# RupertLuo/Valley

Hardware: NVIDIA H100
Metric: generated tokens/s (8-frame video requests: ViT-L/14 encode + pool/project + LLaMA prefill + 256 greedy tokens per sequence) (higher is better)
Workload: dtype bf16

## Files before the change

### include/valley_b200.h

```cpp
#ifndef VALLEY_B200_H_
#define VALLEY_B200_H_

#include <stdint.h>

#ifdef __cplusplus
extern "C" {
#endif

typedef struct vly_ctx vly_ctx;
typedef struct vly_kv vly_kv;

typedef enum {
  VLY_OK = 0,
  VLY_ERR_INVALID = -1,
  VLY_ERR_CUDA = -2,
  VLY_ERR_STATE = -3,
  VLY_ERR_IM_COUNT = -10,
  VLY_ERR_IM_CUT = -11,
  VLY_ERR_INDEX = -12
} vly_status;

typedef enum { VLY_F32 = 0, VLY_BF16 = 1, VLY_F16 = 2 } vly_dtype;

typedef struct {
// ... 103 lines not shown
  float* scores_out;
  float* logits_out;
  int64_t* beam_indices_out;
  int32_t* steps_out;
} vly_beam;

int vly_beam_search(vly_ctx* ctx, vly_kv* kv, const vly_beam* params, const float* first_logits_dev, int prompt_len, int n_steps,
                    int64_t* seq_out_dev, float* scores_out_dev, int* gen_len_out_dev, void* stream);
int vly_kv_beam_reorder(vly_ctx* ctx, vly_kv* kv, const int32_t* parent_rows_dev, int from_pos, void* stream);

int vly_kernel_launch_count(vly_ctx* ctx, int64_t* out);
int vly_held_bytes(int64_t* device_bytes, int64_t* pinned_bytes);
int vly_num_sms(vly_ctx* ctx, int* out);

int vly_kv_debug_counters(vly_kv* kv, long long* host_out, int n);
void vly_set_error_(const char* message);

int vly_test_gemm(vly_ctx* ctx, const void* a_dev, const void* w_dev, int M, int N, int K, int epi, const float* bias_dev,
                  const void* residual_dev, void* out_dev, int block_n, void* stream);
int vly_test_vit_attention(vly_ctx* ctx, const void* qkv_dev, int n_frames, void* out_dev, void* stream);
int vly_test_sample_filter(vly_ctx* ctx, const float* logits_dev, int B, int V, float temperature, int top_k, float top_p,
                           uint8_t* keep_out_dev, void* stream);
int vly_test_stop_strings(vly_ctx* ctx, const vly_sampling* sampling, int V, const int64_t* tokens_dev, int B, int n,
                          uint8_t* out_dev, void* stream);
int vly_test_gemv(vly_ctx* ctx, int mode, const void* w_dev, const void* x_dev, int N, int K, int B, int64_t ldx, float eps,
                  const void* res_dev, void* out_dev, void* kcache_dev, void* vcache_dev, int Smax, int pos, float* logits_dev,
                  int64_t* next_tokens_dev, void* stream);
int vly_test_decode_attention(vly_ctx* ctx, const void* q_dev, const void* kcache_dev, const void* vcache_dev, int B, int nH,
                              int Smax, int len, const uint8_t* key_mask_dev, void* out_dev, void* stream);

// ... 5 lines not shown
```

### valley_b200/_lib.py

```python
from __future__ import annotations

import ctypes as C
import os

_HERE = os.path.dirname(os.path.abspath(__file__))
LIB_PATH = os.environ.get("VLY_LIB_PATH") or os.path.join(_HERE, "lib", "libvalley_b200.so")


class VlyConfig(C.Structure):
    _fields_ = [
        ("hidden_size", C.c_int32), ("num_hidden_layers", C.c_int32), ("num_attention_heads", C.c_int32),
        ("intermediate_size", C.c_int32), ("vocab_size", C.c_int32),
        ("rms_norm_eps", C.c_float), ("rope_theta", C.c_float),
        ("max_position_embeddings", C.c_int32),
        ("vit_hidden", C.c_int32), ("vit_layers", C.c_int32), ("vit_heads", C.c_int32), ("vit_mlp", C.c_int32),
        ("vit_patch", C.c_int32), ("vit_image", C.c_int32),
        ("vit_eps", C.c_float),
        ("mm_vision_select_layer", C.c_int32),
        ("device", C.c_int32),
        ("patch_pooling_method", C.c_int32),
    ]


class VlyTokens(C.Structure):
# ... 78 lines not shown
    "vly_kv_reset": (_i, [_vp, _vp]),
    "vly_kv_set_key_mask": (_i, [_vp, _vp, _i, _vp]),
    "vly_kv_export": (_i, [_vp, _vp, _i, _i, _vp, _vp]),
    "vly_llama_prefill": (_i, [_vp, _vp, _vp, _i, _i, _i, _vp, _vp, _vp]),
    "vly_llama_decode": (_i, [_vp, _vp, _vp, _vp, _vp, _vp]),
    "vly_generate_greedy": (_i, [_vp, _vp, _vp, _i, _vp, _vp]),
    "vly_cross_entropy": (_i, [_vp, _vp, _vp, _i, _i, _i64, _vp, _vp]),
    "vly_sample_logits": (_i, [_vp, _vp, _vp, _p(VlySampling), _vp, _vp]),
    "vly_generate": (_i, [_vp, _vp, _vp, _i, _vp, _p(VlySampling), _vp, _vp]),
    "vly_beam_search": (_i, [_vp, _vp, _p(VlyBeam), _vp, _i, _i, _vp, _vp, _vp, _vp]),
    "vly_kv_beam_reorder": (_i, [_vp, _vp, _vp, _i, _vp]),
    "vly_kernel_launch_count": (_i, [_vp, _p(_i64)]),
    "vly_held_bytes": (_i, [_p(_i64), _p(_i64)]),
    "vly_num_sms": (_i, [_vp, _p(_i)]),
    "vly_kv_debug_counters": (_i, [_vp, _vp, _i]),
    "vly_set_error_": (None, [C.c_char_p]),
    "vly_test_gemm": (_i, [_vp, _vp, _vp, _i, _i, _i, _i, _vp, _vp, _vp, _i, _vp]),
    "vly_test_vit_attention": (_i, [_vp, _vp, _i, _vp, _vp]),
    "vly_test_sample_filter": (_i, [_vp, _vp, _i, _i, C.c_float, _i, C.c_float, _vp, _vp]),
    "vly_test_stop_strings": (_i, [_vp, _p(VlySampling), _i, _vp, _i, _i, _vp, _vp]),
    "vly_test_gemv":(_i, [_vp, _i, _vp, _vp, _i, _i, _i, _i64, C.c_float, _vp, _vp, _vp, _vp, _i, _i, _vp, _vp, _vp]),
    "vly_test_decode_attention": (_i, [_vp, _vp, _vp, _vp, _i, _i, _i, _i, _vp, _vp, _vp]),
}

_lib = None


def load():
    global _lib
    if _lib is not None:
# ... 29 lines not shown
```

### valley_b200/csrc/api.cu

```cuda
#include <cuda_runtime.h>
#include <cuda.h>

#include <algorithm>
#include <atomic>
#include <cmath>
#include <cstdarg>
#include <cstdio>
#include <cstdlib>
#include <cstring>
#include <map>
#include <memory>
#include <mutex>
#include <string>
#include <type_traits>
#include <utility>
#include <vector>

#include "../../include/valley_b200.h"
#include "attention_tc.cuh"
#include "common.cuh"
#include "gemm_tc.cuh"
#include "simt_kernels.cuh"
#include "decode_kernels.cuh"
#include "decode_mega.cuh"
// ... 164 lines not shown
  int* d_step = nullptr;
  Owned<bf16> x, q, attn, hb;
  Owned<float> part_o;
  Owned<float2> part_ml;
  Owned<unsigned int> counters;
  Owned<float> part_val;
  Owned<int> part_idx;
  Owned<float> logits;
  Owned<long long> cur_tokens;
  Owned<long long> gen_tokens;
  int nsplit = 1;
  Owned<PhaseDesc> d_phases;
  StepParams mega = {};
  size_t mega_smem = 0;
  Owned<long long> dbg;
  Owned<SampleState> d_sample;
  bool sample_dirty = false;
  bool filtered = false;
  bool recording = false;
  Owned<uint32_t> key_bits;
  bool masked = false;
  int mask_words() const { return Smax / 32; }
  Owned<BeamState> d_beam;
  Owned<long long> beam_tok;
  Owned<int> beam_bidx;
  Owned<float> beam_div;
  Owned<int> beam_from;
  Owned<uint8_t> stop_buf, stop_stage;
  cudaEvent_t stop_event = nullptr;
  bool stop_ready = false;
// ... 828 lines not shown
  if (!c || !ids || !out || B <= 0 || S <= 0) return fail(VLY_ERR_INVALID, "vly_embed_splice: bad argument");
  if (src_map && (!img_idx || !vis_rows)) return fail(VLY_ERR_INVALID, "vly_embed_splice: src_map given without img_idx / vis_rows");
  std::lock_guard<std::mutex> lk(c->mu);
  if (!c->finalized || !c->has_llm) return fail(VLY_ERR_STATE, "vly_embed_splice: LLM weights not loaded");
  CK(cudaSetDevice(c->cfg.device));
  return launch(c, embed_splice_kernel, {dim3(B * S), dim3(128), 0, (cudaStream_t)stream}, (const long long*)ids, src_map, img_idx, c->embed,
                (const bf16*)vis_rows, rows_per_img, (bf16*)out, nullptr, 0, S, c->cfg.hidden_size, c->cfg.vocab_size);
}

static void mega_smem_layout(const vly_config& g, int bmax, size_t* x_bytes, size_t* misc) {
  const bool tc = bmax > 1;
  const int kmax = g.intermediate_size > g.hidden_size ? g.intermediate_size : g.hidden_size;
  const size_t xs_stride_b = tc ? (size_t)(((kmax * 2 + 127) & ~127) + MegaCfg::PAD_TC) : (size_t)kmax * 2;
  *x_bytes = ((size_t)bmax * xs_stride_b + 127) & ~size_t(127);
  const int nv = (tc ? MegaCfg::ROWS_TC : MegaCfg::ROWS) * bmax;
  *misc = (2 * MegaCfg::MAX_STAGES + 2 * MegaCfg::RED_SLOTS + 2) * 8 + (size_t)MegaCfg::RED_SLOTS * 16 * nv * 4 + (3 + 16) * bmax * 4 + 256;
}
static const size_t kMegaSmem = 226 * 1024;
static const int kMegaDbgCounters = 1024 * 8;

struct DecodeSettings {
  int stage_kb = 0;
  int rows = 0;
  int inflight_kb = 100;
  int stages = 0;
  int inflight = 0;
  int attn_ikeys = 0;
  int l2_hint = 1;
  bool dbg = false;
};
static DecodeSettings read_decode_settings() {
// ... 70 lines not shown
    d.type = PH_ATTN; d.N = 0; d.K = 0; d.W = nullptr; d.x_in = nullptr; d.out = kv->attn; add(d);
    d.type = PH_OPROJ; d.N = H; d.K = H; d.W = w.wo; d.x_in = kv->attn; d.out = kv->x; add(d);
    d.type = PH_GATEUP; d.N = 2 * I; d.K = H; d.W = w.wgu; d.x_in = kv->x; d.out = kv->hb; add(d);
    d.type = PH_DOWN; d.N = H; d.K = I; d.W = w.wdown; d.x_in = kv->hb; d.out = kv->x; add(d);
  }
  {
    PhaseDesc d = {};
    d.type = PH_LOGITS; d.N = V; d.K = H; d.W = c->lm_head; d.x_in = kv->x; d.out = nullptr; add(d);
  }
  stage_bytes = (stage_bytes + 127) & ~127;
  for (PhaseDesc& q : ph) {
    if (q.type == PH_ATTN) continue;
    const int sb = q.rows * (q.kc * 2 + pad);
    q.inflight = (s.inflight_kb * 1024 + sb / 2) / sb;
    if (q.inflight < 2) q.inflight = 2;
  }
  int n_stages = (int)(((long long)kMegaSmem - (long long)x_bytes - (long long)misc) / (long long)stage_bytes);
  if (n_stages > MegaCfg::MAX_STAGES) n_stages = MegaCfg::MAX_STAGES;
  const int cap = s.stages > 0 ? s.stages : 4;
  if (n_stages > cap) n_stages = cap;
  if (n_stages < 2)
    return fail(VLY_ERR_INVALID, "vly_kv_create: activations (B=%d, K=%d) leave no room for the weight ring (%d stages, at least 2 needed)",
                B, std::max(I, H), n_stages);
  if (s.dbg) {
    fprintf(stderr, "[vly] decode ring: B=%d x=%zu B, ring budget %zu B, slot %d B, %d slots fit, %d used;", B, x_bytes, ring_budget,
            stage_bytes, (int)(ring_budget / stage_bytes), n_stages);
    for (int i = 0; i < 5 && i < (int)ph.size(); ++i)
      if (ph[i].type != PH_ATTN) fprintf(stderr, " type%d N=%d K=%d rows=%d kc=%d inflight=%d;", ph[i].type, ph[i].N, ph[i].K, ph[i].rows, ph[i].kc, ph[i].inflight);
    fprintf(stderr, " logits rows=%d kc=%d\n", ph.back().rows, ph.back().kc);
    TRY(kv->dbg.alloc(kMegaDbgCounters * sizeof(long long)));
  }
  TRY(kv->d_phases.alloc(ph.size() * sizeof(PhaseDesc)));
  CK(cudaMemcpy(kv->d_phases, ph.data(), ph.size() * sizeof(PhaseDesc), cudaMemcpyHostToDevice));

  StepParams& p = kv->mega;
  p = {};
  p.phases = kv->d_phases; p.n_phases = (int)ph.size();
  p.B = B; p.H = H; p.nH = nH; p.Smax = kv->Smax; p.V = V;
  p.Kmax = std::max(I, H);
  p.eps = g.rms_norm_eps; p.scale_log2e = 0.08838834764831845f * 1.4426950408889634f;
  p.rope = c->rope; p.seq_len = kv->d_len; p.step = kv->d_step; p.embed = c->embed; p.tokens_in = kv->cur_tokens;
  p.x = kv->x; p.q = kv->q; p.attn = kv->attn;
  p.part_o = kv->part_o; p.part_ml = kv->part_ml; p.attn_counters = kv->counters; p.nsplit = kv->nsplit;
  p.key_bits = kv->key_bits; p.mask_words = kv->mask_words();
  p.logits = kv->logits; p.part_val = kv->part_val; p.part_idx = kv->part_idx;
  p.next_tokens = kv->cur_tokens; p.out_tokens = kv->gen_tokens; p.out_stride = kv->Smax;
  p.sample = kv->d_sample;
  p.grid_counter = kv->counters + (size_t)B * nH + 1;
  p.grid_epoch = p.grid_counter + 1;
  p.n_grid_syncs = p.n_phases + 1;
  p.attn_ikeys = s.attn_ikeys;
  p.n_stages = n_stages;
  p.stage_bytes = stage_bytes;
  p.n_inflight = s.inflight > 0 ? s.inflight : n_stages;
  if (p.n_inflight > n_stages) p.n_inflight = n_stages;
  p.l2_hint = s.l2_hint;
  p.dbg = kv->dbg;
  kv->mega_smem = (size_t)n_stages * stage_bytes + x_bytes + misc;
  return VLY_OK;
}

extern "C" int vly_kv_create(vly_ctx* c, int batch, int max_seq, vly_kv** out) {
  if (!c || !out || batch <= 0 || max_seq <= 0) return fail(VLY_ERR_INVALID, "vly_kv_create: bad argument");
  if (!c->finalized || !c->has_llm) return fail(VLY_ERR_STATE, "vly_kv_create: LLM weights not finalised");
  if (max_seq > c->cfg.max_position_embeddings) return fail(VLY_ERR_INVALID, "vly_kv_create: max_seq %d > max_position_embeddings %d", max_seq, c->cfg.max_position_embeddings);
  CK(cudaSetDevice(c->cfg.device));
  const vly_config& g = c->cfg;
  auto kv = std::make_unique<vly_kv>();
  kv->ctx = c;
  kv->B = batch;
  kv->Smax = (max_seq + 127) / 128 * 128;
  const int H = g.hidden_size, nH = g.num_attention_heads, I = g.intermediate_size, V = g.vocab_size, L = g.num_hidden_layers;
// ... 275 lines not shown
  if (next_tokens_dev) CK(cudaMemcpyAsync(next_tokens_dev, kv->cur_tokens, (size_t)B * 8, cudaMemcpyDeviceToDevice, st));
  kv->host_len = past + S;
  return launch(c, set_int_kernel, {dim3(1), dim3(1), 0, st}, kv->d_len, kv->host_len);
}

extern "C" int vly_kv_debug_counters(vly_kv* kv, long long* host_out, int n) {
  if (!kv || !host_out || n < 0) return fail(VLY_ERR_INVALID, "vly_kv_debug_counters: bad argument");
  if (!kv->dbg)
    return fail(VLY_ERR_STATE, "vly_kv_debug_counters: this cache has no counters (B %d; they need B <= 4 and VLY_MEGA_DBG set when it was created)", kv->B);
  if (n > kMegaDbgCounters) return fail(VLY_ERR_INVALID, "vly_kv_debug_counters: %d values requested, the cache holds %d", n, kMegaDbgCounters);
  CK(cudaSetDevice(kv->ctx->cfg.device));
  CK(cudaMemcpy(host_out, kv->dbg, (size_t)n * sizeof(long long), cudaMemcpyDeviceToHost));
  return VLY_OK;
}

static int launch_decode_mega(vly_ctx* c, vly_kv* kv, bool select, cudaStream_t st) {
  StepParams p = kv->mega;
  p.select = select ? 1 : 0;
  LaunchCfg l = {dim3(c->num_sms), dim3(MegaCfg::THREADS), kv->mega_smem, st};
  l.cooperative = true;
  return with_bmax(kv->B, [&](auto bm) { return launch(c, decode_step_kernel<decltype(bm)::value>, l, p); });
}

static int launch_sample_filter(vly_ctx* c, const float* logits, int B, int V, SampleState* s, const int* seq_len, const int* step,
                                long long* next_tokens, long long* out_tokens, int out_stride, bool filter, bool per_op,
                                uint8_t* keep_out, cudaStream_t st) {
  const size_t smem = filter && (size_t)V * 4 <= (size_t)kFilterStageMaxBytes ? (size_t)V * 4 : 0;
  return launch(c, sample_filter_kernel, {dim3(B), dim3(kFilterThreads), smem, st}, logits, V, s, seq_len, step, next_tokens, out_tokens,
                out_stride, filter ? 1 : 0, per_op ? 1 : 0, keep_out);
}
// ... 515 lines not shown
```

### valley_b200/csrc/decode_mega.cuh

```cuda
#pragma once
#include "common.cuh"
#include "simt_kernels.cuh"
#include "decode_kernels.cuh"
#include "sampling.cuh"

namespace vly {

enum PhaseType : int { PH_QKV = 0, PH_ATTN = 1, PH_OPROJ = 2, PH_GATEUP = 3, PH_DOWN = 4, PH_LOGITS = 5 };

struct PhaseDesc {
  int type, N, K, layer;
  int rows, kc;
  int inflight;
  const __nv_bfloat16* W;
  const __nv_bfloat16* x_in;
  __nv_bfloat16* out;
  __nv_bfloat16* kcache;
  __nv_bfloat16* vcache;
};

struct StepParams {
  const PhaseDesc* phases;
  int n_phases;
  int B, H, nH, Smax, V, Kmax;
  float eps, scale_log2e;
  const float2* rope;
  int* seq_len;
// ... 13 lines not shown
  float* part_val;
  int* part_idx;
  long long* next_tokens;
  long long* out_tokens;
  int out_stride;
  SampleState* sample;
  unsigned int* grid_counter;
  unsigned int* grid_epoch;
  int n_grid_syncs;
  int attn_ikeys;
  int n_stages;
  int stage_bytes;
  int n_inflight;
  int l2_hint;
  long long* dbg;
  int select;
};

struct MegaCfg {
  static constexpr int ROWS = 4;
  static constexpr int ROWS_TC = 8;
  static constexpr int PAD_TC = 64;
  static constexpr int CONSUMERS = 512, THREADS = 576;
  static constexpr int RED_SLOTS = 4;
  static constexpr int MAX_STAGES = 8;
  static constexpr int ATTN_KEYS_MIN = 16;
};

VLY_DEVINL uint4 ldcg_v4(const void* p) {
  uint4 r;
  asm volatile("ld.global.cg.v4.u32 {%0, %1, %2, %3}, [%4];\n" : "=r"(r.x), "=r"(r.y), "=r"(r.z), "=r"(r.w) : "l"(p) : "memory");
  return r;
}
VLY_DEVINL float ldcg_bf16(const __nv_bfloat16* p) {
  unsigned short v;
  asm volatile("ld.global.cg.u16 %0, [%1];\n" : "=h"(v) : "l"(p) : "memory");
  return __uint_as_float((uint32_t)v << 16);
}
VLY_DEVINL void mma_m16n8k16_bf16(float (&d)[4], uint32_t a0, uint32_t a1, uint32_t a2, uint32_t a3, uint32_t b0, uint32_t b1) {
  asm volatile("mma.sync.aligned.m16n8k16.row.col.f32.bf16.bf16.f32 {%0,%1,%2,%3}, {%4,%5,%6,%7}, {%8,%9}, {%0,%1,%2,%3};\n"
               : "+f"(d[0]), "+f"(d[1]), "+f"(d[2]), "+f"(d[3])
               : "r"(a0), "r"(a1), "r"(a2), "r"(a3), "r"(b0), "r"(b1));
}

VLY_DEVINL uint32_t ld_acquire_u32(const unsigned int* p) {
  uint32_t v;
  asm volatile("ld.acquire.gpu.global.u32 %0, [%1];\n" : "=r"(v) : "l"(p) : "memory");
  return v;
}
VLY_DEVINL void fence_proxy_async_global() { asm volatile("fence.proxy.async.global;\n" ::: "memory"); }

VLY_DEVINL void grid_sync_consumers(unsigned int* counter, unsigned int target, int ct) {
  asm volatile("bar.sync 2, 544;" ::: "memory");
  if (ct == 0) {
    asm volatile("red.release.gpu.global.add.u32 [%0], 1;\n" ::"l"(counter) : "memory");
    while ((int)(ld_acquire_u32(counter) - target) < 0) {
    }
  }
  asm volatile("bar.sync 2, 544;" ::: "memory");
}

VLY_DEVINL void mega_attention_phase(const StepParams& p, const PhaseDesc& d, const int cw, const int lane, const int pos) {
  const int len = pos + 1;
  const int n_warps = 16 * (int)gridDim.x;
  int ikeys = p.attn_ikeys;
  if (ikeys == 0) {
    if (p.B * p.nH * ((len + 15) >> 4) <= n_warps) ikeys = 16;
    else
      for (ikeys = 32; ikeys < 256; ikeys += 16)
        if (p.B * p.nH * ((len + ikeys - 1) / ikeys) <= n_warps + n_warps / 20) break;
  }
  const int n_act = (len + ikeys - 1) / ikeys;
  const int items = p.B * p.nH * n_act;
  const int hl = lane & 15, hw = lane >> 4;
// ... 150 lines not shown

VLY_DEVINL void mega_epilogue_prefetch(const StepParams& p, const PhaseDesc& d, const bool ok, const int b, const int n, const int pos,
                                       float& pre0, float& pre1) {
  if (ok) {
    if (d.type == PH_OPROJ || d.type == PH_DOWN) pre0 = ldcg_bf16(d.out + (size_t)b * d.N + n);
    else if (d.type == PH_QKV && n < 2 * p.H) {
      const float2 cs = __ldg(p.rope + (size_t)pos * 64 + ((n & 127) >> 1));
      pre0 = cs.x;
      pre1 = cs.y;
    }
  }
}

template <int BMAX, int NV>
VLY_DEVINL void mega_unit_epilogue(const StepParams& p, const PhaseDesc& d, const int lane, const float t, const bool ok, const int r,
                                   const int b, const int n, const float pre0, const float pre1, const int pos, const float* rstd_s,
                                   float* bestv, int* besti, const bool samp_on, const float samp_it, const uint32_t samp_k0,
                                   const uint32_t samp_k1) {
  constexpr unsigned kMask = (NV == 32) ? 0xffffffffu : ((1u << NV) - 1u);
  if (d.type == PH_OPROJ || d.type == PH_DOWN) {
    if (ok) d.out[(size_t)b * d.N + n] = __float2bfloat16_rn(t + pre0);
  } else if (d.type == PH_LOGITS) {
    const float y = t * rstd_s[b];
    if (ok && p.logits != nullptr) p.logits[(size_t)b * d.N + n] = y;
    float bv = ok ? (samp_on ? sample_score(y, samp_it, samp_k0, samp_k1, n, b, pos) : y) : -INFINITY;
    int bi = n;
#pragma unroll
    for (int o = BMAX; o < NV; o <<= 1) {
      const float ov = __shfl_xor_sync(kMask, bv, o);
      const int oi = __shfl_xor_sync(kMask, bi, o);
      if (ov > bv || (ov == bv && oi < bi)) { bv = ov; bi = oi; }
    }
    if (lane < BMAX && lane < p.B && bv > bestv[lane]) {
      bestv[lane] = bv;
      besti[lane] = bi;
    }
  } else {
    const float mine = t * rstd_s[b];
    const float other = __shfl_xor_sync(kMask, mine, BMAX);
    if ((r & 1) == 0 && ok && n + 1 < d.N) {
      float x0 = mine, x1 = other;
      if (d.type == PH_GATEUP) {
        const float gte = bf16_round(x0), up = bf16_round(x1);
        d.out[(size_t)b * (d.N >> 1) + (n >> 1)] = __float2bfloat16_rn(bf16_round(gte / (1.f + __expf(-gte))) * up);
      } else {
        const int which = n / p.H, nh = n - which * p.H, head = nh >> 7, cidx = nh & 127;
        if (which < 2) {
          const float a = x0 * pre0 - x1 * pre1, c2 = x1 * pre0 + x0 * pre1;
          x0 = a;
          x1 = c2;
        }
        __nv_bfloat16* dst;
        if (which == 0) dst = d.out + (size_t)b * p.H + nh;
// ... 38 lines not shown
  constexpr int ROWS = kTC ? M::ROWS_TC : M::ROWS;
  constexpr int NV = ROWS * BMAX;
  constexpr int PAD = kTC ? M::PAD_TC : 0;
  extern __shared__ uint8_t msm_raw[];
  uint8_t* msm = msm_raw + ((128u - (smem_u32(msm_raw) & 127u)) & 127u);
  uint8_t* ring = msm;
  __nv_bfloat16* xs = reinterpret_cast<__nv_bfloat16*>(ring + (size_t)p.n_stages * p.stage_bytes);
  const int xs_stride = kTC ? (((p.Kmax * 2 + 127) & ~127) + PAD) / 2 : p.Kmax;
  const size_t xs_bytes = ((size_t)BMAX * xs_stride * 2 + 127) & ~size_t(127);
  uint8_t* tail = reinterpret_cast<uint8_t*>(xs) + xs_bytes;
  uint64_t* full_bar = reinterpret_cast<uint64_t*>(tail);
  uint64_t* empty_bar = full_bar + M::MAX_STAGES;
  uint64_t* red_full = empty_bar + M::MAX_STAGES;
  uint64_t* red_empty = red_full + M::RED_SLOTS;
  uint64_t* x_bar = red_empty + M::RED_SLOTS;
  float* red = reinterpret_cast<float*>(x_bar + 2);
  float* rstd_s = red + M::RED_SLOTS * 16 * NV;
  float* bestv = rstd_s + BMAX;
  int* besti = reinterpret_cast<int*>(bestv + BMAX);
  float* wred = reinterpret_cast<float*>(besti + BMAX);

  const int tid = threadIdx.x, warp = tid >> 5, lane = tid & 31;
  if (p.sample->all_done) return;
  if (tid == 0) {
    for (int i = 0; i < p.n_stages; ++i) {
      mbar_init(&full_bar[i], 1);
      mbar_init(&empty_bar[i], 16);
    }
    for (int i = 0; i < M::RED_SLOTS; ++i) {
      mbar_init(&red_full[i], 16);
      mbar_init(&red_empty[i], 1);
    }
    mbar_init(x_bar, 1);
    fence_barrier_init();
  }
  __syncthreads();

  if (warp == 0) {
    if (lane == 0) {
      int st = 0;
      uint32_t ph = 0;
      int wst = 0, issued = 0, confirmed = 0;
      uint32_t wph = 0;
      long long* dbg_p = p.dbg != nullptr ? p.dbg + (size_t)blockIdx.x * 32 : nullptr;
      if (dbg_p != nullptr)
        for (int i = 26; i < 32; ++i) dbg_p[i] = 0;
      const bool hint = p.l2_hint != 0;
      const uint64_t pol_stream = l2_policy_evict_first();
      for (int pi = 0; pi < p.n_phases; ++pi) {
        const PhaseDesc d = p.phases[pi];
        if (d.type == PH_ATTN) continue;
        const int rows_u = d.rows, KCp = d.kc;
        const int row_stride = KCp * 2 + PAD;
        const int n_groups = (d.N + rows_u - 1) / rows_u;
        const int n_slices = (d.K + KCp - 1) / KCp;
        const int infl = min(d.inflight, p.n_inflight);
        long long t_blocked = 0;
        for (int g = blockIdx.x; g < n_groups; g += gridDim.x) {
          const int n0 = g * rows_u;
          const int rows = min(rows_u, d.N - n0);
          for (int s = 0; s < n_slices; ++s) {
            const int kc = min(KCp, d.K - s * KCp);
            const long long t_w = dbg_p != nullptr ? clock64() : 0;
            mbar_wait(&empty_bar[st], ph ^ 1);
            while (issued - confirmed >= infl) {
              mbar_wait(&full_bar[wst], wph);
              if (++wst == p.n_stages) { wst = 0; wph ^= 1; }
              ++confirmed;
            }
            if (dbg_p != nullptr) t_blocked += clock64() - t_w;
            ++issued;
            mbar_expect_tx(&full_bar[st], (uint32_t)rows * kc * 2);
            uint8_t* dst = ring + (size_t)st * p.stage_bytes;
            const __nv_bfloat16* src = d.W + (size_t)n0 * d.K + (size_t)s * KCp;
            if (PAD == 0 && kc == d.K) {
// ... 13 lines not shown
    }
    return;
  }

  const bool is_fin = (warp == 17);
  const int ct = tid - 32;
  const int cw = warp - 1;
  const int pos = *p.seq_len;
  const bool samp_on = p.select && p.sample->enabled != 0;
  const float samp_it = p.sample->inv_temp;
  const uint32_t samp_k0 = p.sample->seed_lo, samp_k1 = p.sample->seed_hi;
  unsigned int sync_no = 0;
  const unsigned int sync_base = *p.grid_epoch * (unsigned int)p.n_grid_syncs * gridDim.x;
  long long t_sync = 0, t_stage = 0, t_loop = 0, t_attn = 0, t0 = clock64();
  long long* dbg_o = (p.dbg != nullptr && ct == 0) ? p.dbg + (size_t)blockIdx.x * 32 : nullptr;
  if (dbg_o != nullptr)
    for (int i = 8; i < 26; ++i) dbg_o[i] = 0;
  {
    if (!is_fin) {
      const int chunks = p.B * (p.H >> 3);
      for (int i = blockIdx.x * M::CONSUMERS + ct; i < chunks; i += gridDim.x * M::CONSUMERS) {
        const int b = i / (p.H >> 3), c = i % (p.H >> 3);
        long long id = p.tokens_in[b];
        id = id < 0 ? 0 : (id >= p.V ? p.V - 1 : id);
        *reinterpret_cast<uint4*>(p.x + (size_t)b * p.H + c * 8) = *reinterpret_cast<const uint4*>(p.embed + (size_t)id * p.H + c * 8);
      }
    } else if (lane < BMAX) {
      bestv[lane] = -INFINITY;
      besti[lane] = 0;
    }
    grid_sync_consumers(p.grid_counter, sync_base + (++sync_no) * gridDim.x, ct);
    t_sync += clock64() - t0;
  }

  int st = 0;
  uint32_t ph = 0, xph = 0;
  unsigned int unit_no = 0;
  for (int pi = 0; pi < p.n_phases; ++pi) {
    const PhaseDesc d = p.phases[pi];
    t0 = clock64();
    if (d.type == PH_ATTN) {
      if (!is_fin) mega_attention_phase(p, d, cw, lane, pos);
      t_attn += clock64() - t0;
      if (dbg_o != nullptr) dbg_o[8 + 3 * PH_ATTN + 1] += clock64() - t0;
    } else {
      const bool norm = (d.type == PH_QKV || d.type == PH_GATEUP || d.type == PH_LOGITS);
      const int rows_u = d.rows, KCp = d.kc;
      const int row_stride = KCp * 2 + PAD;
      if (!is_fin) {
        if (ct == 0) {
          fence_proxy_async_global();
          mbar_expect_tx(x_bar, (uint32_t)p.B * d.K * 2);
          for (int b = 0; b < p.B; ++b) bulk_load_1d(xs + (size_t)b * xs_stride, d.x_in + (size_t)b * d.K, (uint32_t)d.K * 2, x_bar);
        }
        mbar_wait(x_bar, xph);
        if (norm) {
          float sq[BMAX];
#pragma unroll
          for (int b = 0; b < BMAX; ++b) sq[b] = 0.f;
          const int chunks = d.K >> 3;
          for (int c = ct; c < chunks; c += M::CONSUMERS) {
#pragma unroll
            for (int b = 0; b < BMAX; ++b) {
              if (b < p.B) {
                const uint4 w = *reinterpret_cast<const uint4*>(xs + (size_t)b * xs_stride + c * 8);
                const uint32_t ww[4] = {w.x, w.y, w.z, w.w};
#pragma unroll
                for (int i = 0; i < 4; ++i) {
                  const float a = bf16_lo(ww[i]), bb = bf16_hi(ww[i]);
                  sq[b] += a * a + bb * bb;
                }
              }
            }
          }
#pragma unroll
          for (int b = 0; b < BMAX; ++b) {
            const float v = warp_sum(sq[b]);
            if (lane == 0) wred[cw * BMAX + b] = v;
          }
        }
      }
      xph ^= 1;
      if (norm) {
        asm volatile("bar.sync 2, 544;" ::: "memory");
        if (!is_fin && ct < BMAX) {
          float t = 0.f;
          for (int w = 0; w < 16; ++w) t += wred[w * BMAX + ct];
          rstd_s[ct] = rsqrtf(t / d.K + p.eps);
        }
        asm volatile("bar.sync 2, 544;" ::: "memory");
      }
      t_stage += clock64() - t0;
      if (dbg_o != nullptr) dbg_o[8 + 3 * d.type] += clock64() - t0;
      t0 = clock64();
      const int n_groups = (d.N + rows_u - 1) / rows_u;
      const int n_slices = (d.K + KCp - 1) / KCp;
      if (!is_fin) {
        for (int g = blockIdx.x; g < n_groups; g += gridDim.x, ++unit_no) {
          const int n0 = g * rows_u;
          const int rows = min(rows_u, d.N - n0);
          const int slot = unit_no & (M::RED_SLOTS - 1);
          const uint32_t round = (unit_no / M::RED_SLOTS) & 1;
          if constexpr (kTC) {
            const int gq = lane >> 2, tq = lane & 3;
            float dacc[4] = {0.f, 0.f, 0.f, 0.f}, dacc1[4] = {0.f, 0.f, 0.f, 0.f};
            const bool w_ok = gq < rows, x_ok = gq < p.B;
            for (int s = 0; s < n_slices; ++s) {
              const int kc = min(KCp, d.K - s * KCp);
              mbar_wait(&full_bar[st], ph);
              const uint8_t* wrow = ring + (size_t)st * p.stage_bytes + gq * row_stride;
              const __nv_bfloat16* xrow = xs + (size_t)gq * xs_stride + (size_t)s * KCp;
              const int nblk = kc >> 5, bpw = (nblk + 15) >> 4;
              const int kb0 = cw * bpw, kb1 = min(kb0 + bpw, nblk);
#pragma unroll 4
              for (int kb = kb0; kb < kb1; ++kb) {
                const int k = kb << 5;
                uint4 wb = make_uint4(0, 0, 0, 0), xa = make_uint4(0, 0, 0, 0);
                if (w_ok) wb = *reinterpret_cast<const uint4*>(wrow + (k + tq * 8) * 2);
                if (x_ok) xa = *reinterpret_cast<const uint4*>(xrow + k + tq * 8);
                mma_m16n8k16_bf16(dacc, xa.x, 0u, xa.y, 0u, wb.x, wb.y);
                mma_m16n8k16_bf16(dacc1, xa.z, 0u, xa.w, 0u, wb.z, wb.w);
              }
              __syncwarp();
              if (lane == 0) mbar_arrive(&empty_bar[st]);
              if (++st == p.n_stages) { st = 0; ph ^= 1; }
            }
            dacc[0] += dacc1[0];
            dacc[1] += dacc1[1];
            mbar_wait(&red_empty[slot], round ^ 1);
            if (gq < BMAX) {
              float* rp = red + (slot * 16 + cw) * NV;
              rp[(2 * tq) * BMAX + gq] = dacc[0];
              rp[(2 * tq + 1) * BMAX + gq] = dacc[1];
            }
            __syncwarp();
            if (lane == 0) mbar_arrive(&red_full[slot]);
            continue;
          }
          float acc[NV];
#pragma unroll
          for (int i = 0; i < NV; ++i) acc[i] = 0.f;
          for (int s = 0; s < n_slices; ++s) {
            const int kc = min(KCp, d.K - s * KCp);
            mbar_wait(&full_bar[st], ph);
            for (int c8 = ct * 8; c8 < kc; c8 += M::CONSUMERS * 8) {
              const uint8_t* src = ring + (size_t)st * p.stage_bytes + c8 * 2;
              float xf[BMAX][8];
#pragma unroll
              for (int b = 0; b < BMAX; ++b) {
                const uint4 xv = *reinterpret_cast<const uint4*>(xs + (size_t)b * xs_stride + (size_t)s * KCp + c8);
                xf[b][0] = bf16_lo(xv.x); xf[b][1] = bf16_hi(xv.x); xf[b][2] = bf16_lo(xv.y); xf[b][3] = bf16_hi(xv.y);
                xf[b][4] = bf16_lo(xv.z); xf[b][5] = bf16_hi(xv.z); xf[b][6] = bf16_lo(xv.w); xf[b][7] = bf16_hi(xv.w);
              }
#pragma unroll
              for (int r = 0; r < ROWS; ++r) {
                if (r < rows) {
                  const uint4 wv = *reinterpret_cast<const uint4*>(src + r * row_stride);
                  const float wf[8] = {bf16_lo(wv.x), bf16_hi(wv.x), bf16_lo(wv.y), bf16_hi(wv.y),
                                       bf16_lo(wv.z), bf16_hi(wv.z), bf16_lo(wv.w), bf16_hi(wv.w)};
#pragma unroll
                  for (int b = 0; b < BMAX; ++b)
#pragma unroll
                    for (int e = 0; e < 8; ++e) acc[r * BMAX + b] = fmaf(wf[e], xf[b][e], acc[r * BMAX + b]);
                }
              }
            }
            __syncwarp();
            if (lane == 0) mbar_arrive(&empty_bar[st]);
            if (++st == p.n_stages) { st = 0; ph ^= 1; }
          }
          warp_reduce_scatter<NV>(acc, lane);
          mbar_wait(&red_empty[slot], round ^ 1);
          if ((lane & (32 / NV - 1)) == 0) red[(slot * 16 + cw) * NV + lane / (32 / NV)] = acc[0];
          __syncwarp();
          if (lane == 0) mbar_arrive(&red_full[slot]);
        }
      } else {
        for (int g = blockIdx.x; g < n_groups; g += gridDim.x, ++unit_no) {
          const int n0 = g * rows_u;
          const int slot = unit_no & (M::RED_SLOTS - 1);
          const uint32_t round = (unit_no / M::RED_SLOTS) & 1;
          const int r = lane / BMAX, b = lane % BMAX, n = n0 + r;
          const bool ok = lane < NV && r < rows_u && b < p.B && n < d.N;
          float pre0 = 0.f, pre1 = 0.f;
          mega_epilogue_prefetch(p, d, ok, b, n, pos, pre0, pre1);
          mbar_wait(&red_full[slot], round);
          float t = 0.f;
          if (lane < NV) {
#pragma unroll
            for (int w = 0; w < 16; ++w) t += red[(slot * 16 + w) * NV + lane];
          }
          __syncwarp();
          if (lane == 0) mbar_arrive(&red_empty[slot]);
          if (lane < NV)
            mega_unit_epilogue<BMAX, NV>(p, d, lane, t, ok, r, b, n, pre0, pre1, pos, rstd_s, bestv, besti, samp_on, samp_it, samp_k0, samp_k1);
        }
      }
      t_loop += clock64() - t0;
      if (dbg_o != nullptr) dbg_o[8 + 3 * d.type + 1] += clock64() - t0;
    }
    t0 = clock64();
    if (pi == p.n_phases - 1 && is_fin && lane < p.B) {
      p.part_val[(size_t)lane * gridDim.x + blockIdx.x] = bestv[lane];
      p.part_idx[(size_t)lane * gridDim.x + blockIdx.x] = besti[lane];
    }
    grid_sync_consumers(p.grid_counter, sync_base + (++sync_no) * gridDim.x, ct);
    t_sync += clock64() - t0;
    if (dbg_o != nullptr) dbg_o[8 + 3 * d.type + 2] += clock64() - t0;
  }
  if (dbg_o != nullptr) {
    dbg_o[0] = t_sync; dbg_o[1] = t_stage; dbg_o[2] = t_loop; dbg_o[3] = t_attn; dbg_o[4] = 0;
  }

  if (blockIdx.x == 0 && !is_fin) mega_finish_step(p, cw, lane, ct);
}

}
```

Measured before the change: 387.8.

## Overlap activation loads and RMSNorm with GEMV in decode megakernel, balance tail rows

Splits the per-phase activation bulk load into per-K-slice barriers so consumers can start the first unit's GEMV as soon as their slice arrives, instead of waiting for the whole vector. The RMSNorm sum-of-squares moves to after the first unit's reduction and is signalled through a new norm barrier, taking it off the critical path before compute. Row units are reassigned so full rounds use the normal row count and the leftover tail is spread evenly across all SMs, reducing load imbalance in the last round. Also adds globaltimer boundary timestamps for debugging, plus more mbarrier bookkeeping and phase-parity state that has to stay consistent.

```diff
diff --git a/include/valley_b200.h b/include/valley_b200.h
--- a/include/valley_b200.h
+++ b/include/valley_b200.h
@@ -141,6 +141,7 @@
 int vly_num_sms(vly_ctx* ctx, int* out);
 
 int vly_kv_debug_counters(vly_kv* kv, long long* host_out, int n);
+int vly_kv_debug_boundaries(vly_kv* kv, long long* host_out, int n);
 void vly_set_error_(const char* message);
 
 int vly_test_gemm(vly_ctx* ctx, const void* a_dev, const void* w_dev, int M, int N, int K, int epi, const float* bias_dev,
diff --git a/valley_b200/_lib.py b/valley_b200/_lib.py
--- a/valley_b200/_lib.py
+++ b/valley_b200/_lib.py
@@ -116,6 +116,7 @@
     "vly_held_bytes": (_i, [_p(_i64), _p(_i64)]),
     "vly_num_sms": (_i, [_vp, _p(_i)]),
     "vly_kv_debug_counters": (_i, [_vp, _vp, _i]),
+    "vly_kv_debug_boundaries": (_i, [_vp, _vp, _i]),
     "vly_set_error_": (None, [C.c_char_p]),
     "vly_test_gemm": (_i, [_vp, _vp, _vp, _i, _i, _i, _i, _vp, _vp, _vp, _i, _vp]),
     "vly_test_vit_attention": (_i, [_vp, _vp, _i, _vp, _vp]),
diff --git a/valley_b200/csrc/api.cu b/valley_b200/csrc/api.cu
--- a/valley_b200/csrc/api.cu
+++ b/valley_b200/csrc/api.cu
@@ -202,6 +202,8 @@
   StepParams mega = {};
   size_t mega_smem = 0;
   Owned<long long> dbg;
+  Owned<long long> dbg_bnd;
+  size_t dbg_bnd_n = 0;
   Owned<SampleState> d_sample;
   bool sample_dirty = false;
   bool filtered = false;
@@ -1060,7 +1062,8 @@
   const size_t xs_stride_b = tc ? (size_t)(((kmax * 2 + 127) & ~127) + MegaCfg::PAD_TC) : (size_t)kmax * 2;
   *x_bytes = ((size_t)bmax * xs_stride_b + 127) & ~size_t(127);
   const int nv = (tc ? MegaCfg::ROWS_TC : MegaCfg::ROWS) * bmax;
-  *misc = (2 * MegaCfg::MAX_STAGES + 2 * MegaCfg::RED_SLOTS + 2) * 8 + (size_t)MegaCfg::RED_SLOTS * 16 * nv * 4 + (3 + 16) * bmax * 4 + 256;
+  *misc = (2 * MegaCfg::MAX_STAGES + 2 * MegaCfg::RED_SLOTS + MegaCfg::MAX_XSLICES + 1) * 8 + (size_t)MegaCfg::RED_SLOTS * 16 * nv * 4 +
+          (2 + 16) * bmax * 4 + 256;
 }
 static const size_t kMegaSmem = 226 * 1024;
 static const int kMegaDbgCounters = 1024 * 8;
@@ -1161,6 +1164,13 @@
     const int sb = q.rows * (q.kc * 2 + pad);
     q.inflight = (s.inflight_kb * 1024 + sb / 2) / sb;
     if (q.inflight < 2) q.inflight = 2;
+    const int per_round = q.rows * c->num_sms;
+    q.full = q.N / per_round;
+    const int tail = q.N - q.full * per_round;
+    const bool pairs = q.type == PH_QKV || q.type == PH_GATEUP;
+    q.tail_rows = cdiv(tail, c->num_sms);
+    if (pairs) q.tail_rows = (q.tail_rows + 1) & ~1;
+    q.tail_units = tail > 0 ? cdiv(tail, q.tail_rows) : 0;
   }
   int n_stages = (int)(((long long)kMegaSmem - (long long)x_bytes - (long long)misc) / (long long)stage_bytes);
   if (n_stages > MegaCfg::MAX_STAGES) n_stages = MegaCfg::MAX_STAGES;
@@ -1176,6 +1186,9 @@
       if (ph[i].type != PH_ATTN) fprintf(stderr, " type%d N=%d K=%d rows=%d kc=%d inflight=%d;", ph[i].type, ph[i].N, ph[i].K, ph[i].rows, ph[i].kc, ph[i].inflight);
     fprintf(stderr, " logits rows=%d kc=%d\n", ph.back().rows, ph.back().kc);
     TRY(kv->dbg.alloc(kMegaDbgCounters * sizeof(long long)));
+    kv->dbg_bnd_n = (ph.size() + 1) * (size_t)c->num_sms * 4;
+    TRY(kv->dbg_bnd.alloc(kv->dbg_bnd_n * sizeof(long long)));
+    CK(cudaMemset(kv->dbg_bnd, 0, kv->dbg_bnd_n * sizeof(long long)));
   }
   TRY(kv->d_phases.alloc(ph.size() * sizeof(PhaseDesc)));
   CK(cudaMemcpy(kv->d_phases, ph.data(), ph.size() * sizeof(PhaseDesc), cudaMemcpyHostToDevice));
@@ -1203,6 +1216,7 @@
   if (p.n_inflight > n_stages) p.n_inflight = n_stages;
   p.l2_hint = s.l2_hint;
   p.dbg = kv->dbg;
+  p.dbg_bnd = kv->dbg_bnd;
   kv->mega_smem = (size_t)n_stages * stage_bytes + x_bytes + misc;
   return VLY_OK;
 }
@@ -1508,6 +1522,17 @@
   return VLY_OK;
 }
 
+extern "C" int vly_kv_debug_boundaries(vly_kv* kv, long long* host_out, int n) {
+  if (!kv || !host_out || n < 0) return fail(VLY_ERR_INVALID, "vly_kv_debug_boundaries: bad argument");
+  if (!kv->dbg_bnd)
+    return fail(VLY_ERR_STATE, "vly_kv_debug_boundaries: this cache has no timestamps (B %d; they need B <= 4 and VLY_MEGA_DBG set when it was created)", kv->B);
+  if ((size_t)n > kv->dbg_bnd_n)
+    return fail(VLY_ERR_INVALID, "vly_kv_debug_boundaries: %d values requested, the cache holds %zu", n, kv->dbg_bnd_n);
+  CK(cudaSetDevice(kv->ctx->cfg.device));
+  CK(cudaMemcpy(host_out, kv->dbg_bnd, (size_t)n * sizeof(long long), cudaMemcpyDeviceToHost));
+  return VLY_OK;
+}
+
 static int launch_decode_mega(vly_ctx* c, vly_kv* kv, bool select, cudaStream_t st) {
   StepParams p = kv->mega;
   p.select = select ? 1 : 0;
diff --git a/valley_b200/csrc/decode_mega.cuh b/valley_b200/csrc/decode_mega.cuh
--- a/valley_b200/csrc/decode_mega.cuh
+++ b/valley_b200/csrc/decode_mega.cuh
@@ -11,6 +11,9 @@
 struct PhaseDesc {
   int type, N, K, layer;
   int rows, kc;
+  int full;
+  int tail_rows;
+  int tail_units;
   int inflight;
   const __nv_bfloat16* W;
   const __nv_bfloat16* x_in;
@@ -54,6 +57,7 @@
   int n_inflight;
   int l2_hint;
   long long* dbg;
+  long long* dbg_bnd;
   int select;
 };
 
@@ -64,6 +68,7 @@
   static constexpr int CONSUMERS = 512, THREADS = 576;
   static constexpr int RED_SLOTS = 4;
   static constexpr int MAX_STAGES = 8;
+  static constexpr int MAX_XSLICES = 8;
   static constexpr int ATTN_KEYS_MIN = 16;
 };
 
@@ -90,14 +95,61 @@
 }
 VLY_DEVINL void fence_proxy_async_global() { asm volatile("fence.proxy.async.global;\n" ::: "memory"); }
 
-VLY_DEVINL void grid_sync_consumers(unsigned int* counter, unsigned int target, int ct) {
+VLY_DEVINL int mega_unit_count(const PhaseDesc& d) { return d.full + ((int)blockIdx.x < d.tail_units ? 1 : 0); }
+VLY_DEVINL void mega_unit(const PhaseDesc& d, const int u, int& n0, int& rows) {
+  if (u < d.full) {
+    n0 = (u * (int)gridDim.x + (int)blockIdx.x) * d.rows;
+    rows = d.rows;
+  } else {
+    n0 = d.full * (int)gridDim.x * d.rows + (int)blockIdx.x * d.tail_rows;
+    rows = min(d.tail_rows, d.N - n0);
+  }
+}
+
+VLY_DEVINL long long globaltimer_ns() {
+  long long t;
+  asm volatile("mov.u64 %0, %%globaltimer;" : "=l"(t) : : "memory");
+  return t;
+}
+
+VLY_DEVINL void grid_sync_consumers(unsigned int* counter, unsigned int target, int ct, long long* ts) {
   asm volatile("bar.sync 2, 544;" ::: "memory");
   if (ct == 0) {
+    if (ts != nullptr) ts[0] = globaltimer_ns();
     asm volatile("red.release.gpu.global.add.u32 [%0], 1;\n" ::"l"(counter) : "memory");
     while ((int)(ld_acquire_u32(counter) - target) < 0) {
     }
+    if (ts != nullptr) ts[1] = globaltimer_ns();
   }
   asm volatile("bar.sync 2, 544;" ::: "memory");
+}
+
+template <int BMAX>
+VLY_DEVINL void mega_norm_partials(const StepParams& p, const __nv_bfloat16* xs, const int xs_stride, const int K, const int ct,
+                                   const int cw, const int lane, float* wred) {
+  float sq[BMAX];
+#pragma unroll
+  for (int b = 0; b < BMAX; ++b) sq[b] = 0.f;
+  const int chunks = K >> 3;
+  for (int c = ct; c < chunks; c += MegaCfg::CONSUMERS) {
+#pragma unroll
+    for (int b = 0; b < BMAX; ++b) {
+      if (b < p.B) {
+        const uint4 w = *reinterpret_cast<const uint4*>(xs + (size_t)b * xs_stride + c * 8);
+        const uint32_t ww[4] = {w.x, w.y, w.z, w.w};
+#pragma unroll
+        for (int i = 0; i < 4; ++i) {
+          const float a = bf16_lo(ww[i]), bb = bf16_hi(ww[i]);
+          sq[b] += a * a + bb * bb;
+        }
+      }
+    }
+  }
+#pragma unroll
+  for (int b = 0; b < BMAX; ++b) {
+    const float v = warp_sum(sq[b]);
+    if (lane == 0) wred[cw * BMAX + b] = v;
+  }
 }
 
 VLY_DEVINL void mega_attention_phase(const StepParams& p, const PhaseDesc& d, const int cw, const int lane, const int pos) {
@@ -278,14 +330,14 @@
 
 template <int BMAX, int NV>
 VLY_DEVINL void mega_unit_epilogue(const StepParams& p, const PhaseDesc& d, const int lane, const float t, const bool ok, const int r,
-                                   const int b, const int n, const float pre0, const float pre1, const int pos, const float* rstd_s,
+                                   const int b, const int n, const float pre0, const float pre1, const int pos, const float rstd,
                                    float* bestv, int* besti, const bool samp_on, const float samp_it, const uint32_t samp_k0,
                                    const uint32_t samp_k1) {
   constexpr unsigned kMask = (NV == 32) ? 0xffffffffu : ((1u << NV) - 1u);
   if (d.type == PH_OPROJ || d.type == PH_DOWN) {
     if (ok) d.out[(size_t)b * d.N + n] = __float2bfloat16_rn(t + pre0);
   } else if (d.type == PH_LOGITS) {
-    const float y = t * rstd_s[b];
+    const float y = t * rstd;
     if (ok && p.logits != nullptr) p.logits[(size_t)b * d.N + n] = y;
     float bv = ok ? (samp_on ? sample_score(y, samp_it, samp_k0, samp_k1, n, b, pos) : y) : -INFINITY;
     int bi = n;
@@ -300,7 +352,7 @@
       besti[lane] = bi;
     }
   } else {
-    const float mine = t * rstd_s[b];
+    const float mine = t * rstd;
     const float other = __shfl_xor_sync(kMask, mine, BMAX);
     if ((r & 1) == 0 && ok && n + 1 < d.N) {
       float x0 = mine, x1 = other;
@@ -369,9 +421,9 @@
   uint64_t* red_full = empty_bar + M::MAX_STAGES;
   uint64_t* red_empty = red_full + M::RED_SLOTS;
   uint64_t* x_bar = red_empty + M::RED_SLOTS;
-  float* red = reinterpret_cast<float*>(x_bar + 2);
-  float* rstd_s = red + M::RED_SLOTS * 16 * NV;
-  float* bestv = rstd_s + BMAX;
+  uint64_t* norm_bar = x_bar + M::MAX_XSLICES;
+  float* red = reinterpret_cast<float*>(norm_bar + 1);
+  float* bestv = red + M::RED_SLOTS * 16 * NV;
   int* besti = reinterpret_cast<int*>(bestv + BMAX);
   float* wred = reinterpret_cast<float*>(besti + BMAX);
 
@@ -386,7 +438,8 @@
       mbar_init(&red_full[i], 16);
       mbar_init(&red_empty[i], 1);
     }
-    mbar_init(x_bar, 1);
+    for (int i = 0; i < M::MAX_XSLICES; ++i) mbar_init(&x_bar[i], 1);
+    mbar_init(norm_bar, 16);
     fence_barrier_init();
   }
   __syncthreads();
@@ -405,15 +458,15 @@
       for (int pi = 0; pi < p.n_phases; ++pi) {
         const PhaseDesc d = p.phases[pi];
         if (d.type == PH_ATTN) continue;
-        const int rows_u = d.rows, KCp = d.kc;
+        const int KCp = d.kc;
         const int row_stride = KCp * 2 + PAD;
-        const int n_groups = (d.N + rows_u - 1) / rows_u;
+        const int n_units = mega_unit_count(d);
         const int n_slices = (d.K + KCp - 1) / KCp;
         const int infl = min(d.inflight, p.n_inflight);
         long long t_blocked = 0;
-        for (int g = blockIdx.x; g < n_groups; g += gridDim.x) {
-          const int n0 = g * rows_u;
-          const int rows = min(rows_u, d.N - n0);
+        for (int u = 0; u < n_units; ++u) {
+          int n0, rows;
+          mega_unit(d, u, n0, rows);
           for (int s = 0; s < n_slices; ++s) {
             const int kc = min(KCp, d.K - s * KCp);
             const long long t_w = dbg_p != nullptr ? clock64() : 0;
@@ -457,6 +510,7 @@
   const unsigned int sync_base = *p.grid_epoch * (unsigned int)p.n_grid_syncs * gridDim.x;
   long long t_sync = 0, t_stage = 0, t_loop = 0, t_attn = 0, t0 = clock64();
   long long* dbg_o = (p.dbg != nullptr && ct == 0) ? p.dbg + (size_t)blockIdx.x * 32 : nullptr;
+  auto bnd_ts = [&](int k) { return (p.dbg_bnd != nullptr && ct == 0) ? p.dbg_bnd + ((size_t)k * gridDim.x + blockIdx.x) * 4 : nullptr; };
   if (dbg_o != nullptr)
     for (int i = 8; i < 26; ++i) dbg_o[i] = 0;
   {
@@ -472,15 +526,17 @@
       bestv[lane] = -INFINITY;
       besti[lane] = 0;
     }
-    grid_sync_consumers(p.grid_counter, sync_base + (++sync_no) * gridDim.x, ct);
+    grid_sync_consumers(p.grid_counter, sync_base + (++sync_no) * gridDim.x, ct, bnd_ts(0));
     t_sync += clock64() - t0;
   }
 
   int st = 0;
-  uint32_t ph = 0, xph = 0;
+  uint32_t ph = 0;
+  uint32_t xph = 0;
+  uint32_t nph = 0;
   unsigned int unit_no = 0;
+  PhaseDesc d = p.phases[0];
   for (int pi = 0; pi < p.n_phases; ++pi) {
-    const PhaseDesc d = p.phases[pi];
     t0 = clock64();
     if (d.type == PH_ATTN) {
       if (!is_fin) mega_attention_phase(p, d, cw, lane, pos);
@@ -488,68 +544,43 @@
       if (dbg_o != nullptr) dbg_o[8 + 3 * PH_ATTN + 1] += clock64() - t0;
     } else {
       const bool norm = (d.type == PH_QKV || d.type == PH_GATEUP || d.type == PH_LOGITS);
-      const int rows_u = d.rows, KCp = d.kc;
+      const int KCp = d.kc;
       const int row_stride = KCp * 2 + PAD;
-      if (!is_fin) {
-        if (ct == 0) {
-          fence_proxy_async_global();
-          mbar_expect_tx(x_bar, (uint32_t)p.B * d.K * 2);
-          for (int b = 0; b < p.B; ++b) bulk_load_1d(xs + (size_t)b * xs_stride, d.x_in + (size_t)b * d.K, (uint32_t)d.K * 2, x_bar);
-        }
-        mbar_wait(x_bar, xph);
-        if (norm) {
-          float sq[BMAX];
-#pragma unroll
-          for (int b = 0; b < BMAX; ++b) sq[b] = 0.f;
-          const int chunks = d.K >> 3;
-          for (int c = ct; c < chunks; c += M::CONSUMERS) {
-#pragma unroll
-            for (int b = 0; b < BMAX; ++b) {
-              if (b < p.B) {
-                const uint4 w = *reinterpret_cast<const uint4*>(xs + (size_t)b * xs_stride + c * 8);
-                const uint32_t ww[4] = {w.x, w.y, w.z, w.w};
-#pragma unroll
-                for (int i = 0; i < 4; ++i) {
-                  const float a = bf16_lo(ww[i]), bb = bf16_hi(ww[i]);
-                  sq[b] += a * a + bb * bb;
-                }
-              }
-            }
-          }
-#pragma unroll
-          for (int b = 0; b < BMAX; ++b) {
-            const float v = warp_sum(sq[b]);
-            if (lane == 0) wred[cw * BMAX + b] = v;
-          }
-        }
-      }
-      xph ^= 1;
-      if (norm) {
-        asm volatile("bar.sync 2, 544;" ::: "memory");
-        if (!is_fin && ct < BMAX) {
-          float t = 0.f;
-          for (int w = 0; w < 16; ++w) t += wred[w * BMAX + ct];
-          rstd_s[ct] = rsqrtf(t / d.K + p.eps);
-        }
-        asm volatile("bar.sync 2, 544;" ::: "memory");
+      const int n_units = mega_unit_count(d);
+      const int n_slices = (d.K + KCp - 1) / KCp;
+      const bool has_units = n_units > 0;
+      const int n_xb = min(n_slices, M::MAX_XSLICES);
+      if (!is_fin && ct == 0 && has_units) {
+        fence_proxy_async_global();
+        for (int j = 0; j < n_xb; ++j) {
+          const int c0 = j * KCp, nc = (j == n_xb - 1 ? d.K : c0 + KCp) - c0;
+          mbar_expect_tx(&x_bar[j], (uint32_t)p.B * nc * 2);
+          for (int b = 0; b < p.B; ++b)
+            bulk_load_1d(xs + (size_t)b * xs_stride + c0, d.x_in + (size_t)b * d.K + c0, (uint32_t)nc * 2, &x_bar[j]);
+        }
       }
       t_stage += clock64() - t0;
       if (dbg_o != nullptr) dbg_o[8 + 3 * d.type] += clock64() - t0;
       t0 = clock64();
-      const int n_groups = (d.N + rows_u - 1) / rows_u;
-      const int n_slices = (d.K + KCp - 1) / KCp;
       if (!is_fin) {
-        for (int g = blockIdx.x; g < n_groups; g += gridDim.x, ++unit_no) {
-          const int n0 = g * rows_u;
-          const int rows = min(rows_u, d.N - n0);
+        for (int u = 0; u < n_units; ++u, ++unit_no) {
+          int n0, rows;
+          mega_unit(d, u, n0, rows);
           const int slot = unit_no & (M::RED_SLOTS - 1);
           const uint32_t round = (unit_no / M::RED_SLOTS) & 1;
+          const bool first = u == 0;
           if constexpr (kTC) {
             const int gq = lane >> 2, tq = lane & 3;
             float dacc[4] = {0.f, 0.f, 0.f, 0.f}, dacc1[4] = {0.f, 0.f, 0.f, 0.f};
             const bool w_ok = gq < rows, x_ok = gq < p.B;
             for (int s = 0; s < n_slices; ++s) {
               const int kc = min(KCp, d.K - s * KCp);
+              if (first) {
+                const int j = min(s, n_xb - 1);
+                mbar_wait(&x_bar[j], (xph >> j) & 1u);
+                if (s == 0)
+                  if (long long* ts = bnd_ts(pi)) ts[2] = globaltimer_ns();
+              }
               mbar_wait(&full_bar[st], ph);
               const uint8_t* wrow = ring + (size_t)st * p.stage_bytes + gq * row_stride;
               const __nv_bfloat16* xrow = xs + (size_t)gq * xs_stride + (size_t)s * KCp;
@@ -566,6 +597,8 @@
               }
               __syncwarp();
               if (lane == 0) mbar_arrive(&empty_bar[st]);
+              if (s == 0 && first)
+                if (long long* ts = bnd_ts(pi)) ts[3] = globaltimer_ns();
               if (++st == p.n_stages) { st = 0; ph ^= 1; }
             }
             dacc[0] += dacc1[0];
@@ -578,6 +611,11 @@
             }
             __syncwarp();
             if (lane == 0) mbar_arrive(&red_full[slot]);
+            if (norm && first) {
+              mega_norm_partials<BMAX>(p, xs, xs_stride, d.K, ct, cw, lane, wred);
+              __syncwarp();
+              if (lane == 0) mbar_arrive(norm_bar);
+            }
             continue;
           }
           float acc[NV];
@@ -585,6 +623,12 @@
           for (int i = 0; i < NV; ++i) acc[i] = 0.f;
           for (int s = 0; s < n_slices; ++s) {
             const int kc = min(KCp, d.K - s * KCp);
+            if (first) {
+              const int j = min(s, n_xb - 1);
+              mbar_wait(&x_bar[j], (xph >> j) & 1u);
+              if (s == 0)
+                if (long long* ts = bnd_ts(pi)) ts[2] = globaltimer_ns();
+            }
             mbar_wait(&full_bar[st], ph);
             for (int c8 = ct * 8; c8 < kc; c8 += M::CONSUMERS * 8) {
               const uint8_t* src = ring + (size_t)st * p.stage_bytes + c8 * 2;
@@ -610,6 +654,8 @@
             }
             __syncwarp();
             if (lane == 0) mbar_arrive(&empty_bar[st]);
+            if (s == 0 && first)
+              if (long long* ts = bnd_ts(pi)) ts[3] = globaltimer_ns();
             if (++st == p.n_stages) { st = 0; ph ^= 1; }
           }
           warp_reduce_scatter<NV>(acc, lane);
@@ -617,14 +663,21 @@
           if ((lane & (32 / NV - 1)) == 0) red[(slot * 16 + cw) * NV + lane / (32 / NV)] = acc[0];
           __syncwarp();
           if (lane == 0) mbar_arrive(&red_full[slot]);
+          if (norm && first) {
+            mega_norm_partials<BMAX>(p, xs, xs_stride, d.K, ct, cw, lane, wred);
+            __syncwarp();
+            if (lane == 0) mbar_arrive(norm_bar);
+          }
         }
       } else {
-        for (int g = blockIdx.x; g < n_groups; g += gridDim.x, ++unit_no) {
-          const int n0 = g * rows_u;
+        float rstd = 0.f;
+        for (int u = 0; u < n_units; ++u, ++unit_no) {
+          int n0, rows;
+          mega_unit(d, u, n0, rows);
           const int slot = unit_no & (M::RED_SLOTS - 1);
           const uint32_t round = (unit_no / M::RED_SLOTS) & 1;
           const int r = lane / BMAX, b = lane % BMAX, n = n0 + r;
-          const bool ok = lane < NV && r < rows_u && b < p.B && n < d.N;
+          const bool ok = lane < NV && r < rows && b < p.B && n < d.N;
           float pre0 = 0.f, pre1 = 0.f;
           mega_epilogue_prefetch(p, d, ok, b, n, pos, pre0, pre1);
           mbar_wait(&red_full[slot], round);
@@ -635,9 +688,19 @@
           }
           __syncwarp();
           if (lane == 0) mbar_arrive(&red_empty[slot]);
+          if (norm && u == 0) {
+            mbar_wait(norm_bar, nph);
+            float sq = 0.f;
+            for (int w = 0; w < 16; ++w) sq += wred[w * BMAX + b];
+            rstd = rsqrtf(sq / d.K + p.eps);
+          }
           if (lane < NV)
-            mega_unit_epilogue<BMAX, NV>(p, d, lane, t, ok, r, b, n, pre0, pre1, pos, rstd_s, bestv, besti, samp_on, samp_it, samp_k0, samp_k1);
-        }
+            mega_unit_epilogue<BMAX, NV>(p, d, lane, t, ok, r, b, n, pre0, pre1, pos, rstd, bestv, besti, samp_on, samp_it, samp_k0, samp_k1);
+        }
+      }
+      if (has_units) {
+        xph ^= (1u << n_xb) - 1u;
+        if (norm) nph ^= 1u;
       }
       t_loop += clock64() - t0;
       if (dbg_o != nullptr) dbg_o[8 + 3 * d.type + 1] += clock64() - t0;
@@ -647,9 +710,11 @@
       p.part_val[(size_t)lane * gridDim.x + blockIdx.x] = bestv[lane];
       p.part_idx[(size_t)lane * gridDim.x + blockIdx.x] = besti[lane];
     }
-    grid_sync_consumers(p.grid_counter, sync_base + (++sync_no) * gridDim.x, ct);
+    const PhaseDesc dn = p.phases[pi + 1 < p.n_phases ? pi + 1 : pi];
+    grid_sync_consumers(p.grid_counter, sync_base + (++sync_no) * gridDim.x, ct, bnd_ts(pi + 1));
     t_sync += clock64() - t0;
     if (dbg_o != nullptr) dbg_o[8 + 3 * d.type + 2] += clock64() - t0;
+    d = dn;
   }
   if (dbg_o != nullptr) {
     dbg_o[0] = t_sync; dbg_o[1] = t_stage; dbg_o[2] = t_loop; dbg_o[3] = t_attn; dbg_o[4] = 0;
```

Result: no change. 389.5, median of 6 (+0.4%).
